# tgale96/sputnik

Hardware: AMD Instinct MI355X
Metric: effective TFLOP/s (nnz-FLOPs) DSD block=128 M=K=N=4096 @ 1/2/4/8 GPU vs density (higher is better)
Workload: dtype f16

## Files before the change

### sputnik_amd/csrc/dispatch.cpp

```cpp
#include <atomic>
#include <cstdint>
#include <cstdlib>
#include <cstring>
#include <mutex>

#include "api_internal.h"
#include "block_gemm.h"
#include "dsd4w.h"
#include "layout.h"
#include "metadata.h"
#include "sputnik/sputnik.h"
#include "sputnik_amd.h"

namespace sputnik_amd {

static unsigned long long *g_debug = nullptr;

constexpr int kMaxDevices = 64;

static std::atomic<unsigned long long> g_incall_events{0};
static std::atomic<unsigned long long> g_bt_launches{0};
static thread_local int t_product_depth = 0;
struct InProduct {
  InProduct() { ++t_product_depth; }
// ... 443 lines not shown
         (m.data != nullptr || (long long)m.rows * m.cols == 0);
}

bool SparseOk(const BlockMatrix &s) {
  const int b = AsInt(s.block_size);
  if (b != 128) return false;
  if (s.rows < 0 || s.cols < 0 || s.nonzeros < 0) return false;
  if (s.rows % b != 0 || s.cols % b != 0 || s.nonzeros % (b * b) != 0)
    return false;
  if ((s.cols / b) > 32767 || (s.rows / b) > 32767) return false;
  if (s.offsets == nullptr) return false;
  if (s.nonzeros > 0 && (s.data == nullptr || s.indices == nullptr))
    return false;
  return true;
}

bool Aligned8(const MatmulShape &s) {
  return s.m % 8 == 0 && s.n % 8 == 0 && s.k % 8 == 0 && s.m >= 0 &&
         s.n >= 0 && s.k >= 0;
}

bool StrideOk(long long rows_in_tile, long long ld_elems) {
  return rows_in_tile * ld_elems * 2 <= kMaxLaneOffset;
}

Status PrepareDsd(const BlockMatrix &a, bool ta, const Matrix &b, bool tb,
                  const Matrix &c, GemmParams *p, bool *needs_meta) {
  if (a.block_size != BlockSize::k128) return Status::kNotSupported;
  if (!SparseOk(a) || !DenseOk(b) || !DenseOk(c)) return Status::kNoKernel;
  if (!ValidMatmul(a, ta, b, tb, c)) return Status::kNoKernel;
  const MatmulShape s(a, ta, b, tb);
  if (!Aligned8(s)) return Status::kNoKernel;
  const bool d_kc = tb;
  if (!StrideOk(d_kc ? CfgSparse::kBN : 64, s.ldb)) return Status::kNoKernel;
  *needs_meta = ta;
  if (ta && (a.offsets_t == nullptr || a.indices_t == nullptr ||
             a.block_offsets == nullptr))
    return Status::kMissingMetadata;

  *p = GemmParams{};
  p->s_data = static_cast<const char *>(a.data);
  p->s_offsets = static_cast<const int *>(ta ? a.offsets_t : a.offsets);
  p->s_indices = static_cast<const short *>(ta ? a.indices_t : a.indices);
  p->s_block_offsets =
      ta ? static_cast<const int *>(a.block_offsets) : nullptr;
  p->s_blocks = (int)(a.nonzeros / (kBlock * kBlock));
  p->d_data = static_cast<const char *>(b.data);
  p->d_ld = (long long)s.ldb * 2;
  p->c_data = static_cast<char *>(c.data);
  p->c_ld = (long long)s.ldc * 2;
  p->num_rows = s.m / kBM;
  p->num_jtiles = (s.n + CfgSparse::kBN - 1) / CfgSparse::kBN;
  p->j_limit = s.n;
  p->num_tiles = p->num_rows * p->num_jtiles;
  return Status::kOk;
}

Status PrepareDds(const Matrix &a, bool ta, const BlockMatrix &b, bool tb,
                  const Matrix &c, GemmParams *p, bool *needs_meta) {
  if (b.block_size != BlockSize::k128) return Status::kNotSupported;
  if (!SparseOk(b) || !DenseOk(a) || !DenseOk(c)) return Status::kNoKernel;
  if (!ValidMatmul(a, ta, b, tb, c)) return Status::kNoKernel;
  const MatmulShape s(a, ta, b, tb);
  if (!Aligned8(s)) return Status::kNoKernel;
  const bool d_kc = !ta;
  if (!StrideOk(d_kc ? CfgSparse::kBN : 64, s.lda)) return Status::kNoKernel;
  const bool col_order = !tb;
  *needs_meta = col_order;
  if (col_order && (b.offsets_t == nullptr || b.indices_t == nullptr ||
                    b.block_offsets == nullptr))
    return Status::kMissingMetadata;

  *p = GemmParams{};
  p->s_data = static_cast<const char *>(b.data);
  p->s_offsets = static_cast<const int *>(col_order ? b.offsets_t : b.offsets);
  p->s_indices =
      static_cast<const short *>(col_order ? b.indices_t : b.indices);
  p->s_block_offsets =
      col_order ? static_cast<const int *>(b.block_offsets) : nullptr;
  p->d_data = static_cast<const char *>(a.data);
  p->d_ld = (long long)s.lda * 2;
  p->c_data = static_cast<char *>(c.data);
  p->c_ld = (long long)s.ldc * 2;
  p->s_blocks = (int)(b.nonzeros / (kBlock * kBlock));
  p->num_rows = s.n / kBM;
  p->num_jtiles = (s.m + CfgSparse::kBN - 1) / CfgSparse::kBN;
  p->j_limit = s.m;
  p->num_tiles = p->num_rows * p->num_jtiles;
  return Status::kOk;
}

Status PrepareSdd(const Matrix &a, bool ta, const Matrix &b, bool tb,
                  const BlockMatrix &c, GemmParams *p) {
  if (c.block_size != BlockSize::k128) return Status::kNotSupported;
  if (!SparseOk(c) || !DenseOk(a) || !DenseOk(b)) return Status::kNoKernel;
  if (!ValidMatmul(a, ta, b, tb, c)) return Status::kNoKernel;
  const MatmulShape s(a, ta, b, tb);
  if (!Aligned8(s)) return Status::kNoKernel;
  if (!StrideOk(ta ? 64 : 128, s.lda) || !StrideOk(tb ? 128 : 64, s.ldb))
    return Status::kNoKernel;
  const int blocks = c.nonzeros / (kBlock * kBlock);
  if (blocks > 0 && c.row_indices == nullptr)
    return Status::kMissingRowIndices;

  *p = GemmParams{};
  p->s_data = static_cast<const char *>(a.data);
// ... 1081 lines not shown
```

### sputnik_amd/csrc/dsd4w.hip

```cpp
#include <hip/hip_runtime.h>
#include <stdint.h>

#include <cstdlib>

#include "api_internal.h"
#include "block_gemm.h"
#include "dsd4w.h"
#include "dsd4w_asm.inc"

namespace sputnik_amd {
namespace {

constexpr int kRankScratch = 24576;
constexpr uint32_t kOob = 0x80000000u;

struct Pick {
  int row_a, row_b, e_a, n_a, e_b, n_b, target;
  int uniform;
};

__device__ Pick rank_wave(const GemmParams &p, char *lds, int wave, int lane,
                          int ra, int rb, int o0_pre, bool pre) {
  const int R = p.num_rows;
  const int o0 = pre ? o0_pre : lane <= R ? p.s_offsets[lane] : 0;
  const int o1 = __shfl_down(o0, 1, 64);
  const int nr = lane < R ? o1 - o0 : -1;
  int *keys = reinterpret_cast<int *>(lds + kRankScratch + wave * 256);
  int *nbr = reinterpret_cast<int *>(lds + kRankScratch + 2048 + wave * 256);
  const bool live = lane < R;
  const int key = live ? (nr << 6) | (63 - lane) : -1;
  keys[lane] = key;
  int4 k4[16];
#pragma unroll
  for (int j = 0; j < 16; ++j) k4[j] = *reinterpret_cast<const int4 *>(keys + 4 * j);
  int rank = 0;
#pragma unroll
  for (int j = 0; j < 16; ++j)
    rank += (k4[j].x > key) + (k4[j].y > key) + (k4[j].z > key) + (k4[j].w > key);
  const unsigned long long ba = __ballot(live && rank == ra);
  const unsigned long long bb = __ballot(live && rank == rb);
  Pick out;
  out.row_a = __builtin_ctzll(ba);
  out.row_b = __builtin_ctzll(bb);
  out.e_a = __builtin_amdgcn_readlane(o0, out.row_a);
  out.n_a = __builtin_amdgcn_readlane(nr, out.row_a);
  out.e_b = __builtin_amdgcn_readlane(o0, out.row_b);
  out.n_b = __builtin_amdgcn_readlane(nr, out.row_b);
  if (live) nbr[rank] = nr;
  int v = 0;
  if (lane < (R + 1) / 2) {
    const int j = R - 1 - lane;
    v = lane == j ? nbr[lane] : (nbr[lane] + nbr[j] + 1) / 2;
  }
  int vmax = 0;
#pragma unroll
  for (int bit = 15; bit >= 0; --bit) {
    const int cand = vmax | (1 << bit);
    if (__ballot(v >= cand) != 0) vmax = cand;
  }
  out.target = vmax;
  return out;
}

__device__ Pick rank_block(const GemmParams &p, char *lds, int tid, int ra, int rb) {
  const int R = p.num_rows;
  int *offs = reinterpret_cast<int *>(lds + kRankScratch);
  int *n_by_rank = offs + R + 1;
  int *scratch = reinterpret_cast<int *>(lds + kRankScratch + 4096);
  for (int r = tid; r <= R; r += 256) offs[r] = p.s_offsets[r];
  if (tid == 0) {
    scratch[2] = 0;
    scratch[3] = 1;
  }
  __syncthreads();
  const int n0 = offs[1] - offs[0];
  for (int r = tid; r < R; r += 256) {
    const int nr = offs[r + 1] - offs[r];
    if (nr != n0) scratch[3] = 0;
    int rank = 0;
    for (int r2 = 0; r2 < R; ++r2) {
      const int n2 = offs[r2 + 1] - offs[r2];
      rank += (n2 > nr) | ((n2 == nr) & (r2 < r));
    }
    n_by_rank[rank] = nr;
    if (rank == ra) scratch[0] = r;
    if (rank == rb) scratch[1] = r;
  }
  __syncthreads();
  for (int i = tid; i < (R + 1) / 2; i += 256) {
    const int j = R - 1 - i;
    const int v = i == j ? n_by_rank[i] : (n_by_rank[i] + n_by_rank[j] + 1) / 2;
    atomicMax(&scratch[2], v);
  }
  __syncthreads();
  Pick out;
  out.row_a = __builtin_amdgcn_readfirstlane(scratch[0]);
  out.row_b = __builtin_amdgcn_readfirstlane(scratch[1]);
  out.target = __builtin_amdgcn_readfirstlane(scratch[2]);
  out.uniform = __builtin_amdgcn_readfirstlane(scratch[3]);
  out.e_a = __builtin_amdgcn_readfirstlane(offs[out.row_a]);
  out.n_a = __builtin_amdgcn_readfirstlane(offs[out.row_a + 1]) - out.e_a;
  out.e_b = __builtin_amdgcn_readfirstlane(offs[out.row_b]);
  out.n_b = __builtin_amdgcn_readfirstlane(offs[out.row_b + 1]) - out.e_b;
  __syncthreads();
  return out;
}

__device__ __forceinline__ unsigned long long exp_stamp(int dep) {
#if (SPUTNIK_EXP & 512) != 0
  unsigned long long t;
  asm volatile("s_memrealtime %0\n s_waitcnt lgkmcnt(0)"
               : "=s"(t) : "s"(__builtin_amdgcn_readfirstlane(dep)));
  return t;
#else
  (void)dep;
  return 0;
#endif
}

template <bool kBf16, int kEpi, bool kDds, bool kSdd = false, bool kNt = false,
          bool kTt = false, bool kTn = false>
__global__ void __launch_bounds__(256, 1) dsd4w_kernel(const GemmParams p) {
  constexpr bool kWaveEpi = kEpi != 0;
  constexpr bool kDs = kEpi == 3 || kEpi == 4 || kEpi == 5 || kEpi == 6 || kEpi == 7;
  constexpr bool kBar2 = kEpi == 4;
  constexpr bool kKs = kEpi == 6;
  constexpr bool kTp = kEpi == 7;
  static_assert(!kTp || (!kSdd && !kDds && !kNt && !kTt && !kTn), "tall pipeline: DSD NN");
  static_assert(!kDds || kEpi == 1 || kEpi == 3, "DDS: per-wave epilogue only");
  static_assert(!kSdd || ((kEpi == 3 || (kEpi == 4 && !kTt) || (kEpi == 1 && kTn) ||
                           (kKs && !kNt && !kTt && !kTn)) && !kDds),
                "SDD: double slots (TN: per-step images), per-wave epilogue");
  static_assert(!kKs || kSdd, "K-split: SDD NN only");
  constexpr bool kARowsT = (kTt || kTn) && kSdd;
  constexpr bool kDdsTt = kDds && kTt;
  [[maybe_unused]] const unsigned long long t_entry = __builtin_amdgcn_s_memrealtime();
  __shared__ __attribute__((aligned(1024))) char lds[163840];
  const int tid = threadIdx.x;
  const int lane = tid & 63;
  const int wave = __builtin_amdgcn_readfirstlane(tid >> 6);
  const uint32_t lbase =
      (uint32_t)(uintptr_t)((__attribute__((address_space(3))) char *)lds);

  constexpr int kIdxPreload = 1024;
  const int nb_all = p.s_blocks;
  [[maybe_unused]] const unsigned long long t_karg = exp_stamp(nb_all);
  const bool idx_pre = nb_all <= kIdxPreload &&
                       (reinterpret_cast<uintptr_t>(p.s_indices) & 15) == 0;
  typedef unsigned v4u_t __attribute__((ext_vector_type(4)));
  v4u_t idx_lo = {0u, 0u, 0u, 0u}, idx_hi = {0u, 0u, 0u, 0u};
  if (idx_pre) {
    const __amdgpu_buffer_rsrc_t ri = __builtin_amdgcn_make_buffer_rsrc(
        const_cast<short *>(p.s_indices), 0, (nb_all * 2 + 3) & ~3, 0x00020000);
    idx_lo = __builtin_bit_cast(v4u_t, __builtin_amdgcn_raw_buffer_load_b128(
                                            ri, lane * 32, 0, 0));
    idx_hi = __builtin_bit_cast(v4u_t, __builtin_amdgcn_raw_buffer_load_b128(
                                            ri, lane * 32 + 16, 0, 0));
  }
#ifndef SPUTNIK_OFF_EARLY
#define SPUTNIK_OFF_EARLY 1
#endif
  const bool off_early = SPUTNIK_OFF_EARLY && !kSdd && !kTp && p.num_rows < 64;
  int off_pre = 0;
  if (off_early && lane <= p.num_rows) off_pre = p.s_offsets[lane];
  auto kblock_of = [&](int e) {
    if constexpr (kSdd) return e;
    if (!idx_pre || e >= nb_all) return scalar_load_short(p.s_indices, e);
    const int l = e >> 4, d = (e & 15) >> 1;
    const unsigned w0 = __builtin_amdgcn_readlane(idx_lo.x, l);
    const unsigned w1 = __builtin_amdgcn_readlane(idx_lo.y, l);
    const unsigned w2 = __builtin_amdgcn_readlane(idx_lo.z, l);
    const unsigned w3 = __builtin_amdgcn_readlane(idx_lo.w, l);
    const unsigned w4 = __builtin_amdgcn_readlane(idx_hi.x, l);
    const unsigned w5 = __builtin_amdgcn_readlane(idx_hi.y, l);
    const unsigned w6 = __builtin_amdgcn_readlane(idx_hi.z, l);
    const unsigned w7 = __builtin_amdgcn_readlane(idx_hi.w, l);
    const unsigned w = d == 0 ? w0 : d == 1 ? w1 : d == 2 ? w2 : d == 3 ? w3
                     : d == 4 ? w4 : d == 5 ? w5 : d == 6 ? w6 : w7;
    return (int)((e & 1) ? (w >> 16) : (w & 0xffff));
  };

  int srow, j0;
  int b1, n1, b2 = 0, n2 = 0;
  bool producer = false, collect = false;
  int pair_id = 0;
  [[maybe_unused]] unsigned long long t_rank = 0;
  unsigned epoch = p.pair_epoch;
  if (p.pair != 0 && p.pair_sync != nullptr)
    epoch = ((unsigned)scalar_load_int(reinterpret_cast<const int *>(p.pair_sync), 0) &
             0x7fffffffu) + 1u;
  int grp_b0 = 0, grp_count = 0, grp_c = 0;
  bool split_idle = false;
  int kss = 1, kch = 0, kofs = 0;
  unsigned tp_ent = 0, tp_tile = 0, tp_ent2 = 0, tp_tile2 = 0, tp_zero = 0xffffffffu;
  int tp_first = 0, tp_second = 0, tp_nzero = 0;
  if constexpr (kSdd) {
    int tile = xcd_tile(blockIdx.x, gridDim.x);
    const int R = !kKs && p.sdd_tail != 0
                      ? sdd_tail_rows<256>(p, reinterpret_cast<int *>(lds + kRankScratch), tid)
                      : p.num_rows;
    const bool band = p.sdd_order >= 1;
    const int per = band ? ((R + 255) / 256 + 7) & ~7 : (R + 255) / 256;
    const int r0 = min(R, tid * per), r1 = min(R, r0 + per);
    int local = 0, gmin = 0x7fffffff, gmax = 0;
    for (int r = r0; r < r1; ++r) {
      const int gr = (p.c_offsets[r + 1] - p.c_offsets[r] + 3) / 4;
      local += gr;
      gmin = min(gmin, gr);
      gmax = max(gmax, gr);
    }
    int incl = local;
#pragma unroll
    for (int d = 1; d < 64; d <<= 1) {
      const int v = __shfl_up(incl, d, 64);
      if (lane >= d) incl += v;
    }
#pragma unroll
    for (int d = 1; d < 64; d <<= 1) {
      gmin = min(gmin, __shfl_xor(gmin, d, 64));
      gmax = max(gmax, __shfl_xor(gmax, d, 64));
    }
    int *wsum = reinterpret_cast<int *>(lds + kRankScratch);
    if (lane == 63) {
      wsum[wave] = incl;
      wsum[4 + wave] = gmin;
      wsum[8 + wave] = gmax;
    }
    __syncthreads();
    int before = 0, total = 0;
    for (int w2 = 0; w2 < 4; ++w2) {
      const int v = wsum[w2];
      before += w2 < wave ? v : 0;
      total += v;
      gmin = min(gmin, wsum[4 + w2]);
      gmax = max(gmax, wsum[8 + w2]);
    }
    if constexpr (kKs) {
      const int nk = p.k_limit / 128;
      for (int s = 8; s >= 2 && kss == 1; s >>= 1)
        if (s <= p.sdd_ksplit && total * s <= (int)gridDim.x && nk >= 2 * s) kss = s;
      kch = tile / max(total, 1);
      tile -= kch * total;
      if (kch >= kss) tile = total;
    } else {
      tile = (int)blockIdx.x < total ? xcd_tile(blockIdx.x, total) : total;
    }
    int start = before + incl - local;
    const bool uniform = gmin == gmax;
// ... 163 lines not shown
    }
    __syncthreads();
    for (int w2 = 0; w2 < 4; ++w2) {
      if (wk[4 * w2] < k0) { k0 = wk[4 * w2]; m0 = wk[4 * w2 + 1]; }
      if (wk[4 * w2 + 2] < k1) { k1 = wk[4 * w2 + 2]; m1 = wk[4 * w2 + 3]; }
    }
    const long long T = (long long)P * NB;
    const long long b0 = min(T, q0 * NB + m0);
    const long long b1g = w + 1 == G ? T : min(T, q1 * NB + m1);
    const int nblk = (int)min(128LL, max(0LL, b1g - b0));
    auto describe = [&](int x, unsigned &ent, unsigned &til) {
      ent = 0;
      til = 0;
      if (x >= nblk) return;
      const long long g = b0 + x;
      const int q = (int)(g / NB), e = (int)(g - (long long)q * NB);
      int lo = 0, hi = R;
      while (hi - lo > 1) {
        const int mid = (lo + hi) >> 1;
        if (loff[mid] <= e) lo = mid; else hi = mid;
      }
      const bool last = e == loff[lo + 1] - 1;
      ent = (unsigned)e | ((unsigned)q << 24);
      til = (unsigned)lo | ((unsigned)q << 16) | (last ? 0x80000000u : 0u);
    };
    describe(lane, tp_ent, tp_tile);
    describe(64 + lane, tp_ent2, tp_tile2);
    {
      const long long Z = (long long)P * E;
      const int zlo = (int)(Z * sw0 / stot), zhi = (int)(Z * sw1 / stot);
      int *zl = wsc + 48;
      int e = before + incl - local;
      for (int r = r0; r < r1; ++r) {
        if (loff[r + 1] != loff[r]) continue;
        for (int q = 0; q < P; ++q) {
          const long long rank = (long long)q * E + e;
          if (rank >= zlo && rank < zhi) zl[rank - zlo] = r | (q << 16);
        }
        ++e;
      }
      __syncthreads();
      tp_nzero = min(64, zhi - zlo);
      tp_zero = lane < tp_nzero ? (unsigned)zl[lane] : 0xffffffffu;
    }
    __syncthreads();
    j0 = 0;
    srow = 0;
    b1 = 0;
    n1 = nblk;
    tp_first = (int)(__builtin_amdgcn_readlane(tp_ent, 0) & 0xffffffu);
    tp_second = (int)(__builtin_amdgcn_readlane(tp_ent, nblk > 1 ? 1 : 0) & 0xffffffu);
    split_idle = nblk == 0;
  } else if (p.pair != 0 && p.pair_split == 2) {
    const int nt = p.num_tiles;
    const int gch = (int)blockIdx.x >= nt ? 1 : 0;
    const int t = xcd_tile((int)blockIdx.x - gch * nt, nt);
    srow = t % p.num_rows;
    j0 = (t / p.num_rows) * 512;
    const int e_r = scalar_load_int(p.s_offsets, srow);
    const int n_r = scalar_load_int(p.s_offsets, srow + 1) - e_r;
    const int c0 = gch * n_r / 2, c1 = (gch + 1) * n_r / 2;
    b1 = e_r + c0;
    n1 = c1 - c0;
    pair_id = t;
    if (gch == 0) {
      producer = n1 > 0;
      split_idle = n1 == 0;
    } else {
      collect = n_r / 2 > 0;
    }
  } else if (p.pair != 0) {
    const int R = p.num_rows;
    const int half = R >> 1;
    const int n_light = p.num_jtiles * half;
    const int n_solo = p.num_jtiles * (R & 1);
    const int bid = blockIdx.x;
    int role, panel, pi;
    const bool xcd2 = p.pair_xcd2 != 0 && p.num_jtiles == 8 && n_solo == 0 &&
                      (half & 1) == 0;
    const int rot = xcd2 ? xcd_rotation() : 0;
    auto place = [&](int b) {
      if (xcd2) {
        const int x = b & 7, k = b >> 3;
        panel = 2 * (x >> 1) + (k & 1);
        pi = p.pair_xcd2 == 2 ? 2 * (k >> 1) + (x & 1)
           : (fast_xcd(x, rot) ^ (p.pair_xcd2 == 3 ? 1 : 0)) * (half >> 1) + (k >> 1);
      } else {
        const int t = xcd_tile(b, n_light);
        panel = t / half;
        pi = t % half;
      }
    };
    if (bid < n_light) {
      role = 0;
      place(bid);
    } else if (bid < n_light + n_solo) {
      role = 1;
      panel = bid - n_light;
      pi = half;
    } else {
      role = 2;
      place(bid - n_light - n_solo);
    }
    const Pick rp = R < 64 ? rank_wave(p, lds, wave, lane, pi, R - 1 - pi, off_pre, off_early)
                           : rank_block(p, lds, tid, pi, R - 1 - pi);
    t_rank = exp_stamp(rp.target + rp.e_a + rp.e_b);
    const int min_handoff = p.min_handoff > 0 ? p.min_handoff : SPUTNIK_MIN_HANDOFF;
    int hb = role == 1 ? 0 : rp.n_a - rp.target;
    if (hb < min_handoff) hb = 0;
    pair_id = panel * half + pi;
    j0 = panel * 512;
    if (role == 0) {
      srow = rp.row_b;
      b1 = rp.e_a;
      n1 = hb;
      b2 = rp.e_b;
      n2 = rp.n_b;
      producer = hb > 0;
    } else {
      srow = rp.row_a;
      b1 = rp.e_a + hb;
      n1 = rp.n_a - hb;
      collect = hb > 0;
    }
  } else {
    const int tile = xcd_tile(blockIdx.x, gridDim.x);
    const int panel = tile / p.num_rows;
    const int target = tile % p.num_rows;
    j0 = panel * 512;
    if (p.num_rows < 64) {
      const Pick rp = rank_wave(p, lds, wave, lane, target, target, off_pre, off_early);
      srow = rp.row_a;
      b1 = rp.e_a;
      n1 = rp.n_a;
    } else if (p.num_rows <= kLptRows) {
      const Pick rp = rank_block(p, lds, tid, target, target);
      srow = rp.row_a;
      b1 = rp.e_a;
      n1 = rp.n_a;
      const int R = p.num_rows;
      if (p.xcd_rows != 0 && rp.uniform != 0 && (R & 7) == 0 &&
          (int)gridDim.x == p.num_tiles) {
        const int rx = R >> 3, x = (int)blockIdx.x & 7, tx = (int)blockIdx.x >> 3;
        srow = x * rx + tx % rx;
        j0 = (tx / rx) * 512;
        const int *offs = reinterpret_cast<const int *>(lds + kRankScratch);
        b1 = __builtin_amdgcn_readfirstlane(offs[srow]);
      }
    } else {
      srow = target;
      b1 = scalar_load_int(p.s_offsets, srow);
      n1 = scalar_load_int(p.s_offsets, srow + 1) - b1;
    }
  }
  srow = __builtin_amdgcn_readfirstlane(srow);
  j0 = __builtin_amdgcn_readfirstlane(j0);
  const int ntot = n1 + n2;

  typedef unsigned v4u __attribute__((ext_vector_type(4)));
  if (split_idle) {
  } else if (ntot == 0 && kDds) {
    const v4u z = {0u, 0u, 0u, 0u};
    for (int id = tid; id < 512 * 16; id += 256) {
      const int r = id >> 4, cc = id & 15;
      if (j0 + r >= p.j_limit) continue;
      __builtin_nontemporal_store(
          z, reinterpret_cast<v4u *>(p.c_data + (long long)(j0 + r) * p.c_ld +
                                     (long long)srow * 256 + cc * 16));
    }
  } else if (ntot == 0) {
    const v4u z = {0u, 0u, 0u, 0u};
    for (int id = tid; id < 128 * 64; id += 256) {
      const int r = id >> 6, cc = id & 63;
      const int jc = j0 + cc * 8;
      if (jc >= p.j_limit) continue;
      __builtin_nontemporal_store(
          z, reinterpret_cast<v4u *>(p.c_data + ((long long)srow * 128 + r) * p.c_ld +
                                     (long long)jc * 2));
    }
  } else {
    const int b2m = b2 - n1;
    const int xlast = ntot - 1;
    auto entry = [&](int x) { return x + (x < n1 ? b1 : b2m); };
    const int kb0 = kblock_of(kTp ? tp_first : entry(0));
    const int kb1 = kblock_of(kTp ? tp_second : entry(xlast < 1 ? xlast : 1));
    constexpr bool kColOrder =
        !kDdsTt && ((kDds && !kNt) || ((kTn || kTt) && !kSdd));
    const int bo0 = kColOrder ? scalar_load_int(p.s_block_offsets, entry(0)) : 0;
    const int bo1 =
        kColOrder ? scalar_load_int(p.s_block_offsets, entry(xlast < 1 ? xlast : 1)) : 0;
    [[maybe_unused]] const unsigned long long t_kb = exp_stamp(kb0 + kb1);

    uint32_t vs, vs1 = 0;
    if constexpr (!kDdsTt && ((kDds && !kNt) || kTt || kTn)) {
      const int k = 8 * wave + (lane >> 4);
      const int pc = lane & 15;
      const int c = (((pc >> 1) ^ tr_key(k)) << 1) | (pc & 1);
      vs = (uint32_t)(k * (kARowsT ? p.s_ld : 256) + c * 16);
    } else if constexpr (kDs) {
      const long long srs = kSdd ? p.s_ld : 256;
      auto off = [&](int x) {
        const int r = 32 * wave + 8 * x + (lane >> 3);
        return (uint32_t)(r * srs + (((lane & 7) ^ ((r >> 1) & 7)) << 4));
      };
      vs = off(0);
      vs1 = off(1);
    } else {
      const int srow_l = 32 * wave + (lane >> 2);
      vs = (uint32_t)(srow_l * 256 + (((lane & 3) ^ ((srow_l >> 1) & 3)) << 4));
    }
    uint32_t vd[2];
#pragma unroll
    for (int x = 0; x < 2; ++x) {
      if constexpr (!kDdsTt && ((kDds && kDs) || kNt || kTt)) {
        const int r = 8 * x + (lane >> 3);
        vd[x] = j0 + 128 * wave < p.j_limit
                    ? (uint32_t)(r * p.d_ld + (((lane & 7) ^ ((r >> 1) & 7)) << 4))
                    : kOob;
      } else if constexpr (kDds && !kTn && !kDdsTt) {
        const int r = lane >> 2;
        vd[x] = j0 + 128 * wave < p.j_limit
                    ? (uint32_t)(r * p.d_ld + (((lane & 3) ^ ((r >> 1) & 3)) << 4))
                    : kOob;
      } else {
        const int k = (lane >> 4) + 8 * x;
        const int pc = lane & 15;
        const int c = (((pc >> 1) ^ tr_key(k)) << 1) | (pc & 1);
        const int col = (kSdd ? grp_c * 128 : j0 + 128 * wave) + c * 8;
        vd[x] = col < p.j_limit ? (uint32_t)((lane >> 4) * p.d_ld + c * 16) : kOob;
      }
    }
    const uint32_t own = lbase + 32768u + 32768u * wave;
    const int r16 = lane & 15, g = lane >> 4;
    const uint32_t vrs =
        (kDds ? own : lbase) +
        (kDs ? (uint32_t)(r16 * 128 + ((g ^ ((r16 >> 1) & 7)) << 4))
             : (uint32_t)(r16 * 64 + ((g ^ ((r16 >> 1) & 3)) << 4)));
    const uint32_t vrs1 = vrs ^ 64u;
    const int q = (lane >> 2) & 3, pp = lane & 3;
    const int kr = 8 * g + q;
    uint32_t vrd[8];
#pragma unroll
    for (int n = 0; n < 8; ++n)
      vrd[n] = (kDds || kTt ? lbase : own) +
               (uint32_t)(kr * 256 + pp * 8 + ((n ^ tr_key(kr)) << 5));
    uint32_t vrt[8];
#pragma unroll
    for (int m = 0; m < 8; ++m)
      vrt[m] = (kDds ? own : lbase) +
               (uint32_t)(kr * 256 + pp * 8 + ((m ^ tr_key(kr)) << 5));
    const uint32_t vrk0 = (kDds ? lbase : own) +
                          (uint32_t)(r16 * 128 + ((g ^ ((r16 >> 1) & 7)) << 4));
    const uint32_t vrk1 = vrk0 ^ 64u;
    const uint32_t vw0 = lbase + (uint32_t)(r16 * 1040 + (128 * wave + 4 * g) * 2);
    const uint32_t vw1 = vw0 + 64 * 1040;
    const uint32_t wreg = lbase + 32768u + 32768u * wave;
    uint32_t vws[8], vrb[4];
#pragma unroll
    for (int n = 0; n < 8; ++n)
      vws[n] = wreg + (uint32_t)(r16 * 256 + (((2 * n + (g >> 1)) ^ r16) << 4) + 8 * (g & 1));
#pragma unroll
    for (int qq = 0; qq < 4; ++qq) {
      const int rr = 4 * qq + g;
      vrb[qq] = wreg + (uint32_t)(rr * 256 + ((r16 ^ rr) << 4));
    }
    const bool cvalid = kSdd   ? wave < grp_count
                        : kDds ? j0 + 128 * wave < p.j_limit
                               : j0 + 128 * wave + r16 * 8 < p.j_limit;
    const long long cld = kSdd ? 256 : p.c_ld;
    const uint32_t vco = cvalid ? (uint32_t)(g * cld + r16 * 16) : kOob;
    const uint32_t vpl = (uint32_t)(wave * 65536 + lane * 16);
    const uint32_t vcl = (uint32_t)((lane & 15) * p.c_ld + (lane >> 4) * 8);

    auto U = [](uint32_t x) { return (uint32_t)__builtin_amdgcn_readfirstlane((int)x); };
    auto U64 = [&](uint64_t x) {
      return (uint64_t)U((uint32_t)x) | ((uint64_t)U((uint32_t)(x >> 32)) << 32);
    };
    const uint64_t sd = U64((uint64_t)(
        p.s_data + (kARowsT ? (long long)srow * 256
                    : kSdd  ? (long long)srow * 128 * p.s_ld + (long long)kofs * 256 : 0)));
    const uint64_t dt = U64((uint64_t)(
        p.d_data + (kDdsTt ? (long long)(j0 + 128 * wave) * 2
                    : (kNt || kTt) && !kSdd ? (long long)(j0 + 128 * wave) * p.d_ld
                    : kNt || kTt ? (long long)grp_c * 128 * p.d_ld
                    : kSdd ? (long long)grp_c * 256 + (long long)kofs * 128 * p.d_ld
                           : (long long)(j0 + 128 * wave) * (kDds && !kTn ? p.d_ld : 2))));
    const uint64_t ix = U64((uint64_t)p.s_indices);
    const uint64_t pd =
        U64((uint64_t)(p.pair_partials + (long long)pair_id * 128 * 512));
    const uint64_t flag_p =
        U64(kKs ? (uint64_t)(p.ks_flags + pair_id)
            : p.pair != 0 ? (uint64_t)(p.pair_flags + pair_id) : 0);
    const uint64_t err_p = U64((uint64_t)p.pair_error);
    constexpr bool kKcD = !kDdsTt && ((kDds && !kTn) || kNt || kTt);
    const uint32_t k128 = U((uint32_t)(kKcD ? 256 : 128 * p.d_ld));
    const uint32_t k32 = U((uint32_t)(kKcD ? 64 : 32 * p.d_ld));
    const uint32_t k4 = U((uint32_t)(kKcD ? 16 * p.d_ld : 4 * p.d_ld));
    const uint32_t ms =
        U(lbase + ((kDs && (((!kDds || kNt) && !kTt) || kDdsTt)) ? 4096u : 2048u) * wave);
    const uint32_t sk32 = U((uint32_t)(kARowsT ? 32 * p.s_ld : 0));
    const uint32_t sk128 = U((uint32_t)(kARowsT ? 128 * p.s_ld : 0));
    const uint32_t md = U(lbase + 32768u + 32768u * wave);
    const uint32_t flushrem = U(producer ? (uint32_t)n2 : 0xffffffffu);
    const uint32_t pubat = U(producer && n2 > 0 ? (uint32_t)n2 + 1u : 0u);
    const uint32_t publast = U(producer && n2 == 0 ? 1u : 0u);
    const bool clb = collect && ntot >= 3;
    const uint32_t clbf = U(clb ? 2u : 0xffffffffu), clbc = U(clb ? 1u : 0xffffffffu);
    const bool split_first = p.pair != 0 && p.pair_split == 2 && producer;
    const uint32_t flags =
        U((collect ? 1u : 0u) | (!collect && !(producer && n2 == 0) ? 2u : 0u) |
          (p.pair_fault ? 4u : 0u) | (wave == 3 ? 8u : 0u) | (wave == 0 ? 16u : 0u) |
          (split_first ? 32u : 0u) | (kKs && wave >= grp_count ? 64u : 0u));
    const uint64_t cd = U64(
        kSdd ? (uint64_t)(p.c_data + (long long)(grp_b0 + wave) * 32768)
        : kDds ? (uint64_t)(p.c_data + (long long)(j0 + 128 * wave) * p.c_ld +
                          (long long)srow * 256)
             : (uint64_t)(p.c_data + (long long)srow * 128 * p.c_ld +
                          (long long)(j0 + 128 * wave) * 2));
    const uint64_t bo = U64((uint64_t)p.s_block_offsets);
    const uint32_t c4 = U((uint32_t)(4 * cld));
    const uint32_t s16 = U((uint32_t)(kARowsT ? 4 * p.s_ld : kSdd ? 16 * p.s_ld : 0));
    const uint32_t ub1 = U(b1), un1 = U(n1), ub2m = U(b2m), uxlast = U(xlast),
                   untot = U(ntot), ukb0 = U(kb0), ukb1 = U(kb1), uep = U(epoch),
                   ubo0 = U(bo0), ubo1 = U(bo1), ukss = U(kss), ukch = U(kch);
    const uint32_t crow = U((uint32_t)(128 * p.c_ld));
    const uint32_t unz = U((uint32_t)tp_nzero);

#define DSD4W_INPUTS                                                           \
    [sdlo] "s"((uint32_t)sd), [sdhi] "s"((uint32_t)(sd >> 32)),               \
    [dtlo] "s"((uint32_t)dt), [dthi] "s"((uint32_t)(dt >> 32)),               \
    [k128] "s"(k128), [k32] "s"(k32), [k4] "s"(k4),                            \
    [ixlo] "s"((uint32_t)ix), [ixhi] "s"((uint32_t)(ix >> 32)),               \
    [b1] "s"(ub1), [n1] "s"(un1), [b2m] "s"(ub2m), [xlast] "s"(uxlast),        \
    [ntot] "s"(untot), [kb0] "s"(ukb0), [kb1] "s"(ukb1),                       \
    [flushrem] "s"(flushrem),                                                  \
    [pdlo] "s"((uint32_t)pd), [pdhi] "s"((uint32_t)(pd >> 32)),               \
    [flag] "s"(flag_p), [epoch] "s"(uep), [flags] "s"(flags),                  \
    [err] "s"(err_p), [ms] "s"(ms),                                            \
    [md] "s"(md), [vs] "v"(vs), [vd0] "v"(vd[0]), [vd1] "v"(vd[1]),           \
    [vrs] "v"(vrs), [vrd0] "v"(vrd[0]), [vrd1] "v"(vrd[1]),                   \
    [vs1] "v"(vs1), [vrs1] "v"(vrs1), [s16] "s"(s16),                          \
    [vrk0] "v"(vrk0), [vrk1] "v"(vrk1), [sk32] "s"(sk32), [sk128] "s"(sk128),  \
    [vrt0] "v"(vrt[0]), [vrt1] "v"(vrt[1]), [vrt2] "v"(vrt[2]), [vrt3] "v"(vrt[3]), \
    [vrt4] "v"(vrt[4]), [vrt5] "v"(vrt[5]), [vrt6] "v"(vrt[6]), [vrt7] "v"(vrt[7]), \
    [vrd2] "v"(vrd[2]), [vrd3] "v"(vrd[3]), [vrd4] "v"(vrd[4]),               \
    [vrd5] "v"(vrd[5]), [vrd6] "v"(vrd[6]), [vrd7] "v"(vrd[7]),               \
    [vpl] "v"(vpl), [bolo] "s"((uint32_t)bo), [bohi] "s"((uint32_t)(bo >> 32)),  \
    [bo0] "s"(ubo0), [bo1] "s"(ubo1), [pubat] "s"(pubat), [clbf] "s"(clbf),  \
    [clbc] "s"(clbc), [publast] "s"(publast), [kss] "s"(ukss), [kch] "s"(ukch), \
    [vent] "v"(tp_ent), [vtile] "v"(tp_tile), [vent2] "v"(tp_ent2),         \
    [vtile2] "v"(tp_tile2), [vcl] "v"(vcl), [crow] "s"(crow),                \
    [vzero] "v"(tp_zero), [nzero] "s"(unz)
#define DSD4W_OPERANDS : DSD4W_INPUTS
#define DSD4W_OPERANDS_G DSD4W_OPERANDS, [vw0] "v"(vw0), [vw1] "v"(vw1)
#define DSD4W_INPUTS_W                                                         \
  DSD4W_INPUTS, [cdlo] "s"((uint32_t)cd), [cdhi] "s"((uint32_t)(cd >> 32)),  \
      [c4] "s"(c4), [vws0] "v"(vws[0]), [vws1] "v"(vws[1]), [vws2] "v"(vws[2]), \
      [vws3] "v"(vws[3]), [vws4] "v"(vws[4]), [vws5] "v"(vws[5]),               \
      [vws6] "v"(vws[6]), [vws7] "v"(vws[7]), [vrb0] "v"(vrb[0]),               \
      [vrb1] "v"(vrb[1]), [vrb2] "v"(vrb[2]), [vrb3] "v"(vrb[3]), [vco] "v"(vco)
#define DSD4W_OPERANDS_W : DSD4W_INPUTS_W
#define DSD4W_RECORD(ROLE, EXTRA)                                              \
  if (p.debug != nullptr && wave == 0 && lane < 16) {                          \
    unsigned long long v = 0;                                                  \
    v = lane == 0 ? t_entry : v;                                               \
    v = lane == 1 ? t_asm : v;                                                 \
    v = lane == 2 ? r0 : v;                                                    \
    v = lane == 3 ? r1 : v;                                                    \
    v = lane == 4 ? r2 : v;                                                    \
    v = lane == 5 ? (unsigned long long)ntot : v;                              \
    v = lane == 6 ? (ROLE) : v;                                                \
    v = lane == 7 ? (unsigned long long)srow : v;                              \
    v = lane == 8 ? (unsigned long long)n1 : v;                                \
    v = lane == 9 ? r3 : v;                                                    \
    v = lane == 10 ? r4 : v;                                                   \
    v = lane == 11 ? t_karg : v;                                               \
    v = lane == 12 ? t_rank : v;                                               \
    v = lane == 13 ? t_kb : v;                                                 \
    v = lane == 14 ? (EXTRA) : v;                                              \
// ... 402 lines not shown
```

Before: 1180.

## Hoist lane/panel address setup before ranking and prefetch dense operand lines

Moves the per-lane LDS/global address computation and the panel-dependent scalar setup ahead of the row-ranking and offset loads, pinned with empty asm so the compiler cannot sink them, so this ALU work overlaps the latency of the metadata loads. Tile placement is computed once up front, and a warm-up buffer load touches dense-matrix lines for the panel to pull them into cache early. The rank loop skips its second half when there are 32 or fewer rows. The cost is higher register pressure from values held live longer, plus extra memory traffic from the warm loads.

```diff
diff --git a/sputnik_amd/csrc/dispatch.cpp b/sputnik_amd/csrc/dispatch.cpp
--- a/sputnik_amd/csrc/dispatch.cpp
+++ b/sputnik_amd/csrc/dispatch.cpp
@@ -519,6 +519,7 @@
   p->num_rows = s.m / kBM;
   p->num_jtiles = (s.n + CfgSparse::kBN - 1) / CfgSparse::kBN;
   p->j_limit = s.n;
+  p->k_limit = s.k;
   p->num_tiles = p->num_rows * p->num_jtiles;
   return Status::kOk;
 }
diff --git a/sputnik_amd/csrc/dsd4w.hip b/sputnik_amd/csrc/dsd4w.hip
--- a/sputnik_amd/csrc/dsd4w.hip
+++ b/sputnik_amd/csrc/dsd4w.hip
@@ -30,13 +30,17 @@
   const bool live = lane < R;
   const int key = live ? (nr << 6) | (63 - lane) : -1;
   keys[lane] = key;
-  int4 k4[16];
-#pragma unroll
-  for (int j = 0; j < 16; ++j) k4[j] = *reinterpret_cast<const int4 *>(keys + 4 * j);
   int rank = 0;
-#pragma unroll
-  for (int j = 0; j < 16; ++j)
-    rank += (k4[j].x > key) + (k4[j].y > key) + (k4[j].z > key) + (k4[j].w > key);
+  auto count_above = [&](int j0) {
+    int4 k4[8];
+#pragma unroll
+    for (int j = 0; j < 8; ++j) k4[j] = *reinterpret_cast<const int4 *>(keys + 4 * (j0 + j));
+#pragma unroll
+    for (int j = 0; j < 8; ++j)
+      rank += (k4[j].x > key) + (k4[j].y > key) + (k4[j].z > key) + (k4[j].w > key);
+  };
+  count_above(0);
+  if (R > 32) count_above(8);
   const unsigned long long ba = __ballot(live && rank == ra);
   const unsigned long long bb = __ballot(live && rank == rb);
   Pick out;
@@ -142,6 +146,84 @@
   const uint32_t lbase =
       (uint32_t)(uintptr_t)((__attribute__((address_space(3))) char *)lds);
 
+  auto U = [](uint32_t x) { return (uint32_t)__builtin_amdgcn_readfirstlane((int)x); };
+  auto U64 = [&](uint64_t x) {
+    return (uint64_t)U((uint32_t)x) | ((uint64_t)U((uint32_t)(x >> 32)) << 32);
+  };
+  uint32_t vs = 0, vs1 = 0, vrs = 0, vrs1 = 0, vrd[8], vrt[8], vrk0 = 0, vrk1 = 0;
+  uint32_t vw0 = 0, vw1 = 0, vws[8], vrb[4], vpl = 0, vcl = 0;
+  long long cld = 0;
+  uint64_t ix = 0, err_p = 0, bo = 0;
+  uint32_t k128 = 0, k32 = 0, k4 = 0, ms = 0, sk32 = 0, sk128 = 0, md = 0, c4 = 0, s16 = 0,
+           crow = 0;
+  auto lane_ops = [&]() {
+    if constexpr (!kDdsTt && ((kDds && !kNt) || kTt || kTn)) {
+      const int k = 8 * wave + (lane >> 4);
+      const int pc = lane & 15;
+      const int c = (((pc >> 1) ^ tr_key(k)) << 1) | (pc & 1);
+      vs = (uint32_t)(k * (kARowsT ? p.s_ld : 256) + c * 16);
+    } else if constexpr (kDs) {
+      const long long srs = kSdd ? p.s_ld : 256;
+      auto off = [&](int x) {
+        const int r = 32 * wave + 8 * x + (lane >> 3);
+        return (uint32_t)(r * srs + (((lane & 7) ^ ((r >> 1) & 7)) << 4));
+      };
+      vs = off(0);
+      vs1 = off(1);
+    } else {
+      const int srow_l = 32 * wave + (lane >> 2);
+      vs = (uint32_t)(srow_l * 256 + (((lane & 3) ^ ((srow_l >> 1) & 3)) << 4));
+    }
+    const uint32_t own = lbase + 32768u + 32768u * wave;
+    const int r16 = lane & 15, g = lane >> 4;
+    vrs = (kDds ? own : lbase) +
+          (kDs ? (uint32_t)(r16 * 128 + ((g ^ ((r16 >> 1) & 7)) << 4))
+               : (uint32_t)(r16 * 64 + ((g ^ ((r16 >> 1) & 3)) << 4)));
+    vrs1 = vrs ^ 64u;
+    const int q = (lane >> 2) & 3, pp = lane & 3;
+    const int kr = 8 * g + q;
+#pragma unroll
+    for (int n = 0; n < 8; ++n)
+      vrd[n] = (kDds || kTt ? lbase : own) +
+               (uint32_t)(kr * 256 + pp * 8 + ((n ^ tr_key(kr)) << 5));
+#pragma unroll
+    for (int m = 0; m < 8; ++m)
+      vrt[m] = (kDds ? own : lbase) +
+               (uint32_t)(kr * 256 + pp * 8 + ((m ^ tr_key(kr)) << 5));
+    vrk0 = (kDds ? lbase : own) + (uint32_t)(r16 * 128 + ((g ^ ((r16 >> 1) & 7)) << 4));
+    vrk1 = vrk0 ^ 64u;
+    vw0 = lbase + (uint32_t)(r16 * 1040 + (128 * wave + 4 * g) * 2);
+    vw1 = vw0 + 64 * 1040;
+    const uint32_t wreg = lbase + 32768u + 32768u * wave;
+#pragma unroll
+    for (int n = 0; n < 8; ++n)
+      vws[n] = wreg + (uint32_t)(r16 * 256 + (((2 * n + (g >> 1)) ^ r16) << 4) + 8 * (g & 1));
+#pragma unroll
+    for (int qq = 0; qq < 4; ++qq) {
+      const int rr = 4 * qq + g;
+      vrb[qq] = wreg + (uint32_t)(rr * 256 + ((r16 ^ rr) << 4));
+    }
+    vpl = (uint32_t)(wave * 65536 + lane * 16);
+    ms = U(lbase + ((kDs && (((!kDds || kNt) && !kTt) || kDdsTt)) ? 4096u : 2048u) * wave);
+    md = U(lbase + 32768u + 32768u * wave);
+  };
+  auto pin_lane_ops = [&]() {
+    asm volatile("" : "+v"(vs), "+v"(vs1), "+v"(vrs), "+v"(vrs1), "+v"(vrk0), "+v"(vrk1),
+                      "+v"(vw0), "+v"(vw1), "+v"(vpl));
+    asm volatile("" : "+v"(vrd[0]), "+v"(vrd[1]), "+v"(vrd[2]), "+v"(vrd[3]), "+v"(vrd[4]),
+                      "+v"(vrd[5]), "+v"(vrd[6]), "+v"(vrd[7]));
+    asm volatile("" : "+v"(vrt[0]), "+v"(vrt[1]), "+v"(vrt[2]), "+v"(vrt[3]), "+v"(vrt[4]),
+                      "+v"(vrt[5]), "+v"(vrt[6]), "+v"(vrt[7]));
+    asm volatile("" : "+v"(vws[0]), "+v"(vws[1]), "+v"(vws[2]), "+v"(vws[3]), "+v"(vws[4]),
+                      "+v"(vws[5]), "+v"(vws[6]), "+v"(vws[7]), "+v"(vrb[0]), "+v"(vrb[1]),
+                      "+v"(vrb[2]), "+v"(vrb[3]));
+    asm volatile("" : "+s"(ms), "+s"(md));
+  };
+  if constexpr (!kSdd && kEpi != 7) {
+    lane_ops();
+    pin_lane_ops();
+  }
+
   constexpr int kIdxPreload = 1024;
   const int nb_all = p.s_blocks;
   [[maybe_unused]] const unsigned long long t_karg = exp_stamp(nb_all);
@@ -163,6 +245,15 @@
   const bool off_early = SPUTNIK_OFF_EARLY && !kSdd && !kTp && p.num_rows < 64;
   int off_pre = 0;
   if (off_early && lane <= p.num_rows) off_pre = p.s_offsets[lane];
+  constexpr bool kColOrder =
+      !(kDds && kTt) && ((kDds && !kNt) || ((kTn || kTt) && !kSdd));
+  auto block_offset_of = [&](int e) {
+    if constexpr (!kColOrder) {
+      return 0;
+    } else {
+      return scalar_load_int(p.s_block_offsets, e);
+    }
+  };
   auto kblock_of = [&](int e) {
     if constexpr (kSdd) return e;
     if (!idx_pre || e >= nb_all) return scalar_load_short(p.s_indices, e);
@@ -194,6 +285,149 @@
   int kss = 1, kch = 0, kofs = 0;
   unsigned tp_ent = 0, tp_tile = 0, tp_ent2 = 0, tp_tile2 = 0, tp_zero = 0xffffffffu;
   int tp_first = 0, tp_second = 0, tp_nzero = 0;
+
+  constexpr bool kEarlyOps = !kSdd && !kTp;
+  int plc_a = 0, plc_b = 0;
+  int xcd_share = -1;
+  if constexpr (kEarlyOps) {
+    int panel;
+    if (p.pair != 0 && p.pair_split == 2) {
+      const int nt = p.num_tiles;
+      const int gch = (int)blockIdx.x >= nt ? 1 : 0;
+      const int t = xcd_tile((int)blockIdx.x - gch * nt, nt);
+      panel = t / p.num_rows;
+      plc_a = t;
+      plc_b = gch;
+      pair_id = t;
+    } else if (p.pair != 0) {
+      const int R = p.num_rows;
+      const int half = R >> 1;
+      const int n_light = p.num_jtiles * half;
+      const int n_solo = p.num_jtiles * (R & 1);
+      const int bid = blockIdx.x;
+      int role, pi;
+      const bool xcd2 = p.pair_xcd2 != 0 && p.num_jtiles == 8 && n_solo == 0 &&
+                        (half & 1) == 0;
+      const int rot = xcd2 ? xcd_rotation() : 0;
+      auto place = [&](int b) {
+        if (xcd2) {
+          const int x = b & 7, k = b >> 3;
+          panel = 2 * (x >> 1) + (k & 1);
+          pi = p.pair_xcd2 == 2 ? 2 * (k >> 1) + (x & 1)
+             : (fast_xcd(x, rot) ^ (p.pair_xcd2 == 3 ? 1 : 0)) * (half >> 1) + (k >> 1);
+        } else {
+          const int t = xcd_tile(b, n_light);
+          panel = t / half;
+          pi = t % half;
+        }
+      };
+      if (bid < n_light) {
+        role = 0;
+        place(bid);
+      } else if (bid < n_light + n_solo) {
+        role = 1;
+        panel = bid - n_light;
+        pi = half;
+      } else {
+        role = 2;
+        place(bid - n_light - n_solo);
+      }
+      plc_a = role;
+      plc_b = pi;
+      pair_id = panel * half + pi;
+      if (xcd2) xcd_share = ((bid - (role == 2 ? n_light : 0)) >> 4) + (role == 2 ? half >> 1 : 0);
+    } else {
+      const int tile = xcd_tile(blockIdx.x, gridDim.x);
+      panel = tile / p.num_rows;
+      plc_a = tile % p.num_rows;
+    }
+    j0 = __builtin_amdgcn_readfirstlane(panel * 512);
+  }
+
+  auto arg_ops = [&]() {
+    cld = kSdd ? 256 : p.c_ld;
+    vcl = (uint32_t)((lane & 15) * p.c_ld + (lane >> 4) * 8);
+    ix = U64((uint64_t)p.s_indices);
+    err_p = U64((uint64_t)p.pair_error);
+    constexpr bool kKcD = !kDdsTt && ((kDds && !kTn) || kNt || kTt);
+    k128 = U((uint32_t)(kKcD ? 256 : 128 * p.d_ld));
+    k32 = U((uint32_t)(kKcD ? 64 : 32 * p.d_ld));
+    k4 = U((uint32_t)(kKcD ? 16 * p.d_ld : 4 * p.d_ld));
+    sk32 = U((uint32_t)(kARowsT ? 32 * p.s_ld : 0));
+    sk128 = U((uint32_t)(kARowsT ? 128 * p.s_ld : 0));
+    bo = U64((uint64_t)p.s_block_offsets);
+    c4 = U((uint32_t)(4 * cld));
+    s16 = U((uint32_t)(kARowsT ? 4 * p.s_ld : kSdd ? 16 * p.s_ld : 0));
+    crow = U((uint32_t)(128 * p.c_ld));
+  };
+  uint32_t vd[2] = {0u, 0u}, vco = 0;
+  uint64_t dt = 0, pd = 0, flag_p = 0, cd_panel = 0;
+  auto panel_ops = [&]() {
+#pragma unroll
+    for (int x = 0; x < 2; ++x) {
+      if constexpr (!kDdsTt && ((kDds && kDs) || kNt || kTt)) {
+        const int r = 8 * x + (lane >> 3);
+        vd[x] = j0 + 128 * wave < p.j_limit
+                    ? (uint32_t)(r * p.d_ld + (((lane & 7) ^ ((r >> 1) & 7)) << 4))
+                    : kOob;
+      } else if constexpr (kDds && !kTn && !kDdsTt) {
+        const int r = lane >> 2;
+        vd[x] = j0 + 128 * wave < p.j_limit
+                    ? (uint32_t)(r * p.d_ld + (((lane & 3) ^ ((r >> 1) & 3)) << 4))
+                    : kOob;
+      } else {
+        const int k = (lane >> 4) + 8 * x;
+        const int pc = lane & 15;
+        const int c = (((pc >> 1) ^ tr_key(k)) << 1) | (pc & 1);
+        const int col = (kSdd ? grp_c * 128 : j0 + 128 * wave) + c * 8;
+        vd[x] = col < p.j_limit ? (uint32_t)((lane >> 4) * p.d_ld + c * 16) : kOob;
+      }
+    }
+    const int r16 = lane & 15, g = lane >> 4;
+    const bool cvalid = kSdd   ? wave < grp_count
+                        : kDds ? j0 + 128 * wave < p.j_limit
+                               : j0 + 128 * wave + r16 * 8 < p.j_limit;
+    vco = cvalid ? (uint32_t)(g * cld + r16 * 16) : kOob;
+    dt = U64((uint64_t)(
+        p.d_data + (kDdsTt ? (long long)(j0 + 128 * wave) * 2
+                    : (kNt || kTt) && !kSdd ? (long long)(j0 + 128 * wave) * p.d_ld
+                    : kNt || kTt ? (long long)grp_c * 128 * p.d_ld
+                    : kSdd ? (long long)grp_c * 256 + (long long)kofs * 128 * p.d_ld
+                           : (long long)(j0 + 128 * wave) * (kDds && !kTn ? p.d_ld : 2))));
+    cd_panel = U64(
+        kSdd ? (uint64_t)(p.c_data + (long long)(grp_b0 + wave) * 32768)
+        : kDds ? (uint64_t)(p.c_data + (long long)(j0 + 128 * wave) * p.c_ld)
+               : (uint64_t)(p.c_data + (long long)(j0 + 128 * wave) * 2));
+    pd = U64((uint64_t)(p.pair_partials + (long long)pair_id * 128 * 512));
+    flag_p = U64(kKs ? (uint64_t)(p.ks_flags + pair_id)
+                 : p.pair != 0 ? (uint64_t)(p.pair_flags + pair_id) : 0);
+  };
+  auto pin_panel_ops = [&]() {
+    asm volatile("" : "+v"(vd[0]), "+v"(vd[1]), "+v"(vco), "+v"(vcl));
+    asm volatile("" : "+s"(dt), "+s"(pd), "+s"(flag_p), "+s"(cd_panel));
+  };
+#ifndef SPUTNIK_WARM
+#define SPUTNIK_WARM 1
+#endif
+  [[maybe_unused]] unsigned warm = 0;
+  constexpr bool kWarm = SPUTNIK_WARM != 0 && kEarlyOps && !kDds && !kNt && !kTt && !kTn;
+  if constexpr (kWarm) {
+    const bool on = xcd_share >= 0 && p.k_limit > 0;
+    const int line = xcd_share * 256 + tid;
+    const int col = j0 * 2 + (line & 7) * 128;
+    const long long ext = (long long)(p.k_limit - 1) * p.d_ld + (long long)p.j_limit * 2;
+    const long long off = (long long)(line >> 3) * p.d_ld + col;
+    const __amdgpu_buffer_rsrc_t rw = __builtin_amdgcn_make_buffer_rsrc(
+        const_cast<char *>(p.d_data), 0,
+        !on ? 0 : (int)(ext < 0x7fffffffLL ? ext : 0x7fffffffLL), 0x00020000);
+    warm = __builtin_amdgcn_raw_buffer_load_b32(
+        rw, on && col < p.j_limit * 2 && off < 0x7fffffffLL ? (uint32_t)off : kOob, 0, 0);
+  }
+  if constexpr (kEarlyOps) {
+    arg_ops();
+    panel_ops();
+    pin_panel_ops();
+  }
   if constexpr (kSdd) {
     int tile = xcd_tile(blockIdx.x, gridDim.x);
     const int R = !kKs && p.sdd_tail != 0
@@ -463,17 +697,13 @@
     tp_second = (int)(__builtin_amdgcn_readlane(tp_ent, nblk > 1 ? 1 : 0) & 0xffffffu);
     split_idle = nblk == 0;
   } else if (p.pair != 0 && p.pair_split == 2) {
-    const int nt = p.num_tiles;
-    const int gch = (int)blockIdx.x >= nt ? 1 : 0;
-    const int t = xcd_tile((int)blockIdx.x - gch * nt, nt);
+    const int t = plc_a, gch = plc_b;
     srow = t % p.num_rows;
-    j0 = (t / p.num_rows) * 512;
     const int e_r = scalar_load_int(p.s_offsets, srow);
     const int n_r = scalar_load_int(p.s_offsets, srow + 1) - e_r;
     const int c0 = gch * n_r / 2, c1 = (gch + 1) * n_r / 2;
     b1 = e_r + c0;
     n1 = c1 - c0;
-    pair_id = t;
     if (gch == 0) {
       producer = n1 > 0;
       split_idle = n1 == 0;
@@ -482,45 +712,13 @@
     }
   } else if (p.pair != 0) {
     const int R = p.num_rows;
-    const int half = R >> 1;
-    const int n_light = p.num_jtiles * half;
-    const int n_solo = p.num_jtiles * (R & 1);
-    const int bid = blockIdx.x;
-    int role, panel, pi;
-    const bool xcd2 = p.pair_xcd2 != 0 && p.num_jtiles == 8 && n_solo == 0 &&
-                      (half & 1) == 0;
-    const int rot = xcd2 ? xcd_rotation() : 0;
-    auto place = [&](int b) {
-      if (xcd2) {
-        const int x = b & 7, k = b >> 3;
-        panel = 2 * (x >> 1) + (k & 1);
-        pi = p.pair_xcd2 == 2 ? 2 * (k >> 1) + (x & 1)
-           : (fast_xcd(x, rot) ^ (p.pair_xcd2 == 3 ? 1 : 0)) * (half >> 1) + (k >> 1);
-      } else {
-        const int t = xcd_tile(b, n_light);
-        panel = t / half;
-        pi = t % half;
-      }
-    };
-    if (bid < n_light) {
-      role = 0;
-      place(bid);
-    } else if (bid < n_light + n_solo) {
-      role = 1;
-      panel = bid - n_light;
-      pi = half;
-    } else {
-      role = 2;
-      place(bid - n_light - n_solo);
-    }
+    const int role = plc_a, pi = plc_b;
     const Pick rp = R < 64 ? rank_wave(p, lds, wave, lane, pi, R - 1 - pi, off_pre, off_early)
                            : rank_block(p, lds, tid, pi, R - 1 - pi);
     t_rank = exp_stamp(rp.target + rp.e_a + rp.e_b);
     const int min_handoff = p.min_handoff > 0 ? p.min_handoff : SPUTNIK_MIN_HANDOFF;
     int hb = role == 1 ? 0 : rp.n_a - rp.target;
     if (hb < min_handoff) hb = 0;
-    pair_id = panel * half + pi;
-    j0 = panel * 512;
     if (role == 0) {
       srow = rp.row_b;
       b1 = rp.e_a;
@@ -535,10 +733,7 @@
       collect = hb > 0;
     }
   } else {
-    const int tile = xcd_tile(blockIdx.x, gridDim.x);
-    const int panel = tile / p.num_rows;
-    const int target = tile % p.num_rows;
-    j0 = panel * 512;
+    const int target = plc_a;
     if (p.num_rows < 64) {
       const Pick rp = rank_wave(p, lds, wave, lane, target, target, off_pre, off_early);
       srow = rp.row_a;
@@ -554,7 +749,9 @@
           (int)gridDim.x == p.num_tiles) {
         const int rx = R >> 3, x = (int)blockIdx.x & 7, tx = (int)blockIdx.x >> 3;
         srow = x * rx + tx % rx;
-        j0 = (tx / rx) * 512;
+        j0 = __builtin_amdgcn_readfirstlane((tx / rx) * 512);
+        panel_ops();
+        pin_panel_ops();
         const int *offs = reinterpret_cast<const int *>(lds + kRankScratch);
         b1 = __builtin_amdgcn_readfirstlane(offs[srow]);
       }
@@ -595,123 +792,18 @@
     auto entry = [&](int x) { return x + (x < n1 ? b1 : b2m); };
     const int kb0 = kblock_of(kTp ? tp_first : entry(0));
     const int kb1 = kblock_of(kTp ? tp_second : entry(xlast < 1 ? xlast : 1));
-    constexpr bool kColOrder =
-        !kDdsTt && ((kDds && !kNt) || ((kTn || kTt) && !kSdd));
-    const int bo0 = kColOrder ? scalar_load_int(p.s_block_offsets, entry(0)) : 0;
-    const int bo1 =
-        kColOrder ? scalar_load_int(p.s_block_offsets, entry(xlast < 1 ? xlast : 1)) : 0;
+    const int bo0 = block_offset_of(entry(0));
+    const int bo1 = block_offset_of(entry(xlast < 1 ? xlast : 1));
     [[maybe_unused]] const unsigned long long t_kb = exp_stamp(kb0 + kb1);
 
-    uint32_t vs, vs1 = 0;
-    if constexpr (!kDdsTt && ((kDds && !kNt) || kTt || kTn)) {
-      const int k = 8 * wave + (lane >> 4);
-      const int pc = lane & 15;
-      const int c = (((pc >> 1) ^ tr_key(k)) << 1) | (pc & 1);
-      vs = (uint32_t)(k * (kARowsT ? p.s_ld : 256) + c * 16);
-    } else if constexpr (kDs) {
-      const long long srs = kSdd ? p.s_ld : 256;
-      auto off = [&](int x) {
-        const int r = 32 * wave + 8 * x + (lane >> 3);
-        return (uint32_t)(r * srs + (((lane & 7) ^ ((r >> 1) & 7)) << 4));
-      };
-      vs = off(0);
-      vs1 = off(1);
-    } else {
-      const int srow_l = 32 * wave + (lane >> 2);
-      vs = (uint32_t)(srow_l * 256 + (((lane & 3) ^ ((srow_l >> 1) & 3)) << 4));
-    }
-    uint32_t vd[2];
-#pragma unroll
-    for (int x = 0; x < 2; ++x) {
-      if constexpr (!kDdsTt && ((kDds && kDs) || kNt || kTt)) {
-        const int r = 8 * x + (lane >> 3);
-        vd[x] = j0 + 128 * wave < p.j_limit
-                    ? (uint32_t)(r * p.d_ld + (((lane & 7) ^ ((r >> 1) & 7)) << 4))
-                    : kOob;
-      } else if constexpr (kDds && !kTn && !kDdsTt) {
-        const int r = lane >> 2;
-        vd[x] = j0 + 128 * wave < p.j_limit
-                    ? (uint32_t)(r * p.d_ld + (((lane & 3) ^ ((r >> 1) & 3)) << 4))
-                    : kOob;
-      } else {
-        const int k = (lane >> 4) + 8 * x;
-        const int pc = lane & 15;
-        const int c = (((pc >> 1) ^ tr_key(k)) << 1) | (pc & 1);
-        const int col = (kSdd ? grp_c * 128 : j0 + 128 * wave) + c * 8;
-        vd[x] = col < p.j_limit ? (uint32_t)((lane >> 4) * p.d_ld + c * 16) : kOob;
-      }
-    }
-    const uint32_t own = lbase + 32768u + 32768u * wave;
-    const int r16 = lane & 15, g = lane >> 4;
-    const uint32_t vrs =
-        (kDds ? own : lbase) +
-        (kDs ? (uint32_t)(r16 * 128 + ((g ^ ((r16 >> 1) & 7)) << 4))
-             : (uint32_t)(r16 * 64 + ((g ^ ((r16 >> 1) & 3)) << 4)));
-    const uint32_t vrs1 = vrs ^ 64u;
-    const int q = (lane >> 2) & 3, pp = lane & 3;
-    const int kr = 8 * g + q;
-    uint32_t vrd[8];
-#pragma unroll
-    for (int n = 0; n < 8; ++n)
-      vrd[n] = (kDds || kTt ? lbase : own) +
-               (uint32_t)(kr * 256 + pp * 8 + ((n ^ tr_key(kr)) << 5));
-    uint32_t vrt[8];
-#pragma unroll
-    for (int m = 0; m < 8; ++m)
-      vrt[m] = (kDds ? own : lbase) +
-               (uint32_t)(kr * 256 + pp * 8 + ((m ^ tr_key(kr)) << 5));
-    const uint32_t vrk0 = (kDds ? lbase : own) +
-                          (uint32_t)(r16 * 128 + ((g ^ ((r16 >> 1) & 7)) << 4));
-    const uint32_t vrk1 = vrk0 ^ 64u;
-    const uint32_t vw0 = lbase + (uint32_t)(r16 * 1040 + (128 * wave + 4 * g) * 2);
-    const uint32_t vw1 = vw0 + 64 * 1040;
-    const uint32_t wreg = lbase + 32768u + 32768u * wave;
-    uint32_t vws[8], vrb[4];
-#pragma unroll
-    for (int n = 0; n < 8; ++n)
-      vws[n] = wreg + (uint32_t)(r16 * 256 + (((2 * n + (g >> 1)) ^ r16) << 4) + 8 * (g & 1));
-#pragma unroll
-    for (int qq = 0; qq < 4; ++qq) {
-      const int rr = 4 * qq + g;
-      vrb[qq] = wreg + (uint32_t)(rr * 256 + ((r16 ^ rr) << 4));
-    }
-    const bool cvalid = kSdd   ? wave < grp_count
-                        : kDds ? j0 + 128 * wave < p.j_limit
-                               : j0 + 128 * wave + r16 * 8 < p.j_limit;
-    const long long cld = kSdd ? 256 : p.c_ld;
-    const uint32_t vco = cvalid ? (uint32_t)(g * cld + r16 * 16) : kOob;
-    const uint32_t vpl = (uint32_t)(wave * 65536 + lane * 16);
-    const uint32_t vcl = (uint32_t)((lane & 15) * p.c_ld + (lane >> 4) * 8);
-
-    auto U = [](uint32_t x) { return (uint32_t)__builtin_amdgcn_readfirstlane((int)x); };
-    auto U64 = [&](uint64_t x) {
-      return (uint64_t)U((uint32_t)x) | ((uint64_t)U((uint32_t)(x >> 32)) << 32);
-    };
+    if constexpr (!kEarlyOps) {
+      lane_ops();
+      arg_ops();
+      panel_ops();
+    }
     const uint64_t sd = U64((uint64_t)(
         p.s_data + (kARowsT ? (long long)srow * 256
                     : kSdd  ? (long long)srow * 128 * p.s_ld + (long long)kofs * 256 : 0)));
-    const uint64_t dt = U64((uint64_t)(
-        p.d_data + (kDdsTt ? (long long)(j0 + 128 * wave) * 2
-                    : (kNt || kTt) && !kSdd ? (long long)(j0 + 128 * wave) * p.d_ld
-                    : kNt || kTt ? (long long)grp_c * 128 * p.d_ld
-                    : kSdd ? (long long)grp_c * 256 + (long long)kofs * 128 * p.d_ld
-                           : (long long)(j0 + 128 * wave) * (kDds && !kTn ? p.d_ld : 2))));
-    const uint64_t ix = U64((uint64_t)p.s_indices);
-    const uint64_t pd =
-        U64((uint64_t)(p.pair_partials + (long long)pair_id * 128 * 512));
-    const uint64_t flag_p =
-        U64(kKs ? (uint64_t)(p.ks_flags + pair_id)
-            : p.pair != 0 ? (uint64_t)(p.pair_flags + pair_id) : 0);
-    const uint64_t err_p = U64((uint64_t)p.pair_error);
-    constexpr bool kKcD = !kDdsTt && ((kDds && !kTn) || kNt || kTt);
-    const uint32_t k128 = U((uint32_t)(kKcD ? 256 : 128 * p.d_ld));
-    const uint32_t k32 = U((uint32_t)(kKcD ? 64 : 32 * p.d_ld));
-    const uint32_t k4 = U((uint32_t)(kKcD ? 16 * p.d_ld : 4 * p.d_ld));
-    const uint32_t ms =
-        U(lbase + ((kDs && (((!kDds || kNt) && !kTt) || kDdsTt)) ? 4096u : 2048u) * wave);
-    const uint32_t sk32 = U((uint32_t)(kARowsT ? 32 * p.s_ld : 0));
-    const uint32_t sk128 = U((uint32_t)(kARowsT ? 128 * p.s_ld : 0));
-    const uint32_t md = U(lbase + 32768u + 32768u * wave);
     const uint32_t flushrem = U(producer ? (uint32_t)n2 : 0xffffffffu);
     const uint32_t pubat = U(producer && n2 > 0 ? (uint32_t)n2 + 1u : 0u);
     const uint32_t publast = U(producer && n2 == 0 ? 1u : 0u);
@@ -723,19 +815,14 @@
           (p.pair_fault ? 4u : 0u) | (wave == 3 ? 8u : 0u) | (wave == 0 ? 16u : 0u) |
           (split_first ? 32u : 0u) | (kKs && wave >= grp_count ? 64u : 0u));
     const uint64_t cd = U64(
-        kSdd ? (uint64_t)(p.c_data + (long long)(grp_b0 + wave) * 32768)
-        : kDds ? (uint64_t)(p.c_data + (long long)(j0 + 128 * wave) * p.c_ld +
-                          (long long)srow * 256)
-             : (uint64_t)(p.c_data + (long long)srow * 128 * p.c_ld +
-                          (long long)(j0 + 128 * wave) * 2));
-    const uint64_t bo = U64((uint64_t)p.s_block_offsets);
-    const uint32_t c4 = U((uint32_t)(4 * cld));
-    const uint32_t s16 = U((uint32_t)(kARowsT ? 4 * p.s_ld : kSdd ? 16 * p.s_ld : 0));
+        cd_panel + (kSdd ? 0ull
+                    : kDds ? (uint64_t)((long long)srow * 256)
+                           : (uint64_t)((long long)srow * 128 * p.c_ld)));
     const uint32_t ub1 = U(b1), un1 = U(n1), ub2m = U(b2m), uxlast = U(xlast),
                    untot = U(ntot), ukb0 = U(kb0), ukb1 = U(kb1), uep = U(epoch),
                    ubo0 = U(bo0), ubo1 = U(bo1), ukss = U(kss), ukch = U(kch);
-    const uint32_t crow = U((uint32_t)(128 * p.c_ld));
     const uint32_t unz = U((uint32_t)tp_nzero);
+    if constexpr (kWarm) asm volatile("" ::"v"(warm));
 
 #define DSD4W_INPUTS                                                           \
     [sdlo] "s"((uint32_t)sd), [sdhi] "s"((uint32_t)(sd >> 32)),               \
```

New measurement: 1191, median of 6. Within noise of the previous version (+0.9%).
